# ai4ce/V2X-Sim

Measured on AMD Instinct MI355X. Metric: BEV frames/sec, V2VNet 5-agent detection (256x256 BEV), higher is better.
Workload: dtype bf16

## Files before the change

### v2x-sim_amd/csrc/conv_halo.hip

```cpp
#include "common.h"
#include <cstdlib>

static __device__ __attribute__((aligned(64))) unsigned int g_zero_page_h[16];

typedef const __attribute__((address_space(1))) void *gptr_t;
typedef __attribute__((address_space(3))) void *lptr_t;

__device__ __forceinline__ void glds16h(const void *g, char *lds_wave_base) {
    __builtin_amdgcn_global_load_lds((gptr_t)g, (lptr_t)lds_wave_base, 16, 0, 0);
}

struct HaloArgs {
    const uint16_t *in0;
    const uint16_t *in1;
    const uint32_t *bits;
    int zbits;
    int N, H, W;
    const uint16_t *w;
    const float *scale, *shift;
    int relu;
    void *out;
    int out_cstride, out_coff;
    const uint16_t *w2;
    const float *scale2, *shift2;
// ... 300 lines not shown
            auto hidden = [&](const f32x4_t &lo, const f32x4_t &hi, const float4 &s0, const float4 &t0, const float4 &s1, const float4 &t1) {
                uint4 p;
                p.x = pack_bf16x2(lo[0] * s0.x + t0.x, lo[1] * s0.y + t0.y);
                p.y = pack_bf16x2(lo[2] * s0.z + t0.z, lo[3] * s0.w + t0.w);
                p.z = pack_bf16x2(hi[0] * s1.x + t1.x, hi[1] * s1.y + t1.y);
                p.w = pack_bf16x2(hi[2] * s1.z + t1.z, hi[3] * s1.w + t1.w);
                p.x = v2x_relu_bf16x2_floor(p.x, relu_floor);
                p.y = v2x_relu_bf16x2_floor(p.y, relu_floor);
                p.z = v2x_relu_bf16x2_floor(p.z, relu_floor);
                p.w = v2x_relu_bf16x2_floor(p.w, relu_floor);
                return __builtin_bit_cast(bf16x8_t, p);
            };
            const float4 det_sc0 = *reinterpret_cast<const float4 *>(a.scale + 8 * fq), det_sf0 = *reinterpret_cast<const float4 *>(a.shift + 8 * fq);
            const float4 det_sc1 = *reinterpret_cast<const float4 *>(a.scale + 8 * fq + 4), det_sf1 = *reinterpret_cast<const float4 *>(a.shift + 8 * fq + 4);
            const float4 det_s2 = *reinterpret_cast<const float4 *>(a.scale2 + fq * 4), det_t2 = *reinterpret_cast<const float4 *>(a.shift2 + fq * 4);
            float4 cl[4];
            unsigned long long any_f[4];
#pragma unroll
            for (int f = 0; f < 4; ++f) {
                const bf16x8_t hb0 = hidden(acc[0][f], acc[1][f], det_sc0, det_sf0, det_sc1, det_sf1);
                const f32x4_t d = __builtin_amdgcn_mfma_f32_16x16x32_bf16(wdet[0], hb0, (f32x4_t){0.f, 0.f, 0.f, 0.f}, 0, 0, 0);
                cl[f] = make_float4(d[0] * det_s2.x + det_t2.x, d[1] * det_s2.y + det_t2.y, d[2] * det_s2.z + det_t2.z, d[3] * det_s2.w + det_t2.w);
                const bool maybe = fq < 3 && ((cl[f].y - cl[f].x >= a.det_margin) || (cl[f].w - cl[f].z >= a.det_margin));
                any_f[f] = __builtin_amdgcn_ballot_w64(maybe);
            }
            if ((any_f[0] | any_f[1] | any_f[2] | any_f[3]) != 0) {
                const float4 sc2 = *reinterpret_cast<const float4 *>(a.scale + 32 + 8 * fq), sf2 = *reinterpret_cast<const float4 *>(a.shift + 32 + 8 * fq);
                const float4 sc3 = *reinterpret_cast<const float4 *>(a.scale + 36 + 8 * fq), sf3 = *reinterpret_cast<const float4 *>(a.shift + 36 + 8 * fq);
                float4 s2v[3], t2v[3];
#pragma unroll
                for (int t = 0; t < 3; ++t) {
                    s2v[t] = *reinterpret_cast<const float4 *>(a.scale2 + (t + 1) * 16 + fq * 4);
                    t2v[t] = *reinterpret_cast<const float4 *>(a.shift2 + (t + 1) * 16 + fq * 4);
                }
#pragma unroll
                for (int f = 0; f < 4; ++f) {
                    const float4 c = cl[f];
                    if (any_f[f] == 0) continue;
                    const int r = f >> 1, ch = f & 1;
                    f32x4_t g2 = (f32x4_t){0.f, 0.f, 0.f, 0.f}, g3 = g2;
#pragma unroll
                    for (int kx = 0; kx < 3; ++kx)
#pragma unroll
                        for (int ky = 0; ky < 3; ++ky) {
                            const int kslot = (ky * 3 + kx) * SPP1 + fq;
                            const int pr = 2 * wave + r + ky, pc = ch * 16 + fj + kx;
                            const bf16x8_t Bf = *reinterpret_cast<const bf16x8_t *>(pb + NS0 * 16 + ((pr * PW + pc) * SPP1 + swz<SPP1>(fq, pc)) * 16);
                            const bf16x8_t A2 = *reinterpret_cast<const bf16x8_t *>(s_w + (kslot * COUT + 32 + fj) * 16);
                            const bf16x8_t A3 = *reinterpret_cast<const bf16x8_t *>(s_w + (kslot * COUT + 48 + fj) * 16);
                            g2 = __builtin_amdgcn_mfma_f32_16x16x32_bf16(A2, Bf, g2, 0, 0, 0);
                            g3 = __builtin_amdgcn_mfma_f32_16x16x32_bf16(A3, Bf, g3, 0, 0, 0);
                        }
                    const bf16x8_t hb1 = hidden(g2, g3, sc2, sf2, sc3, sf3);
                    float4 cd[3];
#pragma unroll
                    for (int t = 0; t < 3; ++t) {
                        const f32x4_t e = __builtin_amdgcn_mfma_f32_16x16x32_bf16(wdet[t + 1], hb1, (f32x4_t){0.f, 0.f, 0.f, 0.f}, 0, 0, 0);
                        cd[t] = make_float4(e[0] * s2v[t].x + t2v[t].x, e[1] * s2v[t].y + t2v[t].y, e[2] * s2v[t].z + t2v[t].z, e[3] * s2v[t].w + t2v[t].w);
                    }
                    if (fq < 3) {
                        const int y = ty * TH + 2 * wave + r, x = tx * TW + ch * 16 + fj;
                        const float c0[2] = {c.x, c.z}, c1[2] = {c.y, c.w};
                        const float code[2][6] = {{cd[0].x, cd[0].y, cd[0].z, cd[0].w, cd[1].x, cd[1].y},
                                                  {cd[1].z, cd[1].w, cd[2].x, cd[2].y, cd[2].z, cd[2].w}};
#pragma unroll
                        for (int u = 0; u < 2; ++u) {
                            const float mx = fmaxf(c0[u], c1[u]);
                            const float e0 = expf(c0[u] - mx), e1 = expf(c1[u] - mx);
                            const float fg = e1 / (e0 + e1);
                            if (fg >= a.det_thr) {
                                const int pos = atomicAdd(&a.det_counts[n], 1);
                                if (pos < a.det_cap) {
                                    const unsigned m = (unsigned)((y * a.W + x) * 6 + 2 * fq + u);
                                    reinterpret_cast<unsigned long long *>(a.out)[(size_t)n * a.det_cap + pos] =
                                        ((unsigned long long)(~__float_as_uint(fg)) << 32) | (m << 12) | (unsigned)pos;
                                    float *co = reinterpret_cast<float *>(a.out2) + ((size_t)n * a.det_cap + pos) * 6;
                                    *reinterpret_cast<float2 *>(co) = make_float2(code[u][0], code[u][1]);
                                    *reinterpret_cast<float2 *>(co + 2) = make_float2(code[u][2], code[u][3]);
                                    *reinterpret_cast<float2 *>(co + 4) = make_float2(code[u][4], code[u][5]);
                                }
                            }
                        }
                    }
                }
            }
        } else if constexpr (COUT2 == 0) {
            if (a.x4) {
#pragma unroll
                for (int i = 0; i < TCO; i += 2) {
                    float4 sc[2], sf[2];
#pragma unroll
                    for (int h = 0; h < 2; ++h) {
                        sc[h] = *reinterpret_cast<const float4 *>(s_ss + (i + h) * 16 + fq * 4);
                        sf[h] = *reinterpret_cast<const float4 *>(s_ss + COUT + (i + h) * 16 + fq * 4);
                    }
#pragma unroll
                    for (int f = 0; f < 4; ++f) {
                        const int y = ty * TH + 2 * wave + (f >> 1), x = tx * TW + (f & 1) * 16 + fj;
                        uint32_t ox[2], oy[2];
#pragma unroll
                        for (int h = 0; h < 2; ++h) {
                            ox[h] = v2x_relu_bf16x2_floor(pack_bf16x2(acc[i + h][f][0] * sc[h].x + sf[h].x, acc[i + h][f][1] * sc[h].y + sf[h].y), relu_floor);
                            oy[h] = v2x_relu_bf16x2_floor(pack_bf16x2(acc[i + h][f][2] * sc[h].z + sf[h].z, acc[i + h][f][3] * sc[h].w + sf[h].w), relu_floor);
                        }
                        v2x_store_pair_x4(reinterpret_cast<uint16_t *>(a.out) + ((size_t)(n * a.H + y) * a.W + x) * a.out_cstride + a.out_coff + i * 16 + fq * 4, fq,
                                          ox[0], oy[0], ox[1], oy[1]);
                    }
                }
            } else
#pragma unroll
            for (int i = 0; i < TCO; ++i) {
                const int co = i * 16 + fq * 4;
                const float4 sc = *reinterpret_cast<const float4 *>(s_ss + co);
                const float4 sf = *reinterpret_cast<const float4 *>(s_ss + COUT + co);
#pragma unroll
                for (int f = 0; f < 4; ++f) {
                    const int y = ty * TH + 2 * wave + (f >> 1), x = tx * TW + (f & 1) * 16 + fj;
                    float v0 = acc[i][f][0] * sc.x + sf.x, v1 = acc[i][f][1] * sc.y + sf.y;
                    float v2 = acc[i][f][2] * sc.z + sf.z, v3 = acc[i][f][3] * sc.w + sf.w;
                    uint2 o;
                    o.x = pack_bf16x2(v0, v1);
                    o.y = pack_bf16x2(v2, v3);
                    o.x = v2x_relu_bf16x2_floor(o.x, relu_floor);
                    o.y = v2x_relu_bf16x2_floor(o.y, relu_floor);
                    uint16_t *dst = reinterpret_cast<uint16_t *>(a.out) +
                                    ((size_t)(n * a.H + y) * a.W + x) * a.out_cstride + a.out_coff + co;
                    *reinterpret_cast<uint2 *>(dst) = o;
                }
            }
        } else {
            float4 sc[TCO], sf[TCO];
#pragma unroll
            for (int i = 0; i < TCO; ++i) {
                const int kappa = 32 * (i >> 1) + 8 * fq + 4 * (i & 1);
                sc[i] = *reinterpret_cast<const float4 *>(a.scale + kappa);
                sf[i] = *reinterpret_cast<const float4 *>(a.shift + kappa);
            }
            float4 s2v[TCO2 > 0 ? TCO2 : 1], t2v[TCO2 > 0 ? TCO2 : 1];
#pragma unroll
            for (int i2 = 0; i2 < TCO2; ++i2) {
                s2v[i2] = *reinterpret_cast<const float4 *>(a.scale2 + i2 * 16 + fq * 4);
                t2v[i2] = *reinterpret_cast<const float4 *>(a.shift2 + i2 * 16 + fq * 4);
            }
#pragma unroll
            for (int f = 0; f < 4; ++f) {
                bf16x8_t hb[COUT / 32];
#pragma unroll
                for (int s = 0; s < COUT / 32; ++s) {
                    float h[8];
#pragma unroll
                    for (int half = 0; half < 2; ++half) {
                        const int i = 2 * s + half;
                        h[half * 4 + 0] = acc[i][f][0] * sc[i].x + sf[i].x;
                        h[half * 4 + 1] = acc[i][f][1] * sc[i].y + sf[i].y;
                        h[half * 4 + 2] = acc[i][f][2] * sc[i].z + sf[i].z;
                        h[half * 4 + 3] = acc[i][f][3] * sc[i].w + sf[i].w;
                    }
                    uint4 p;
                    p.x = pack_bf16x2(h[0], h[1]);
                    p.y = pack_bf16x2(h[2], h[3]);
                    p.z = pack_bf16x2(h[4], h[5]);
                    p.w = pack_bf16x2(h[6], h[7]);
                    p.x = v2x_relu_bf16x2_floor(p.x, relu_floor);
                    p.y = v2x_relu_bf16x2_floor(p.y, relu_floor);
                    p.z = v2x_relu_bf16x2_floor(p.z, relu_floor);
                    p.w = v2x_relu_bf16x2_floor(p.w, relu_floor);
                    hb[s] = __builtin_bit_cast(bf16x8_t, p);
                }
                const int y = ty * TH + 2 * wave + (f >> 1), x = tx * TW + (f & 1) * 16 + fj;
                const size_t pix = (size_t)(n * a.H + y) * a.W + x;
#pragma unroll
                for (int i2 = 0; i2 < TCO2; ++i2) {
                    f32x4_t d = (f32x4_t){0.f, 0.f, 0.f, 0.f};
#pragma unroll
                    for (int s = 0; s < COUT / 32; ++s)
                        d = __builtin_amdgcn_mfma_f32_16x16x32_bf16(w2f[i2][s], hb[s], d, 0, 0, 0);
                    const int co = i2 * 16 + fq * 4;
                    if (co >= a.cout2_real) continue;
                    const float4 s2 = s2v[i2], t2 = t2v[i2];
                    float v0 = d[0] * s2.x + t2.x, v1 = d[1] * s2.y + t2.y, v2 = d[2] * s2.z + t2.z, v3 = d[3] * s2.w + t2.w;
                    if (a.relu2) {
                        v0 = fmaxf(v0, 0.f);
                        v1 = fmaxf(v1, 0.f);
                        v2 = fmaxf(v2, 0.f);
                        v3 = fmaxf(v3, 0.f);
                    }
                    if constexpr (EPI2 == 2) {
                        const bool second = a.split > 0 && co >= a.split;
                        float *dst = second ? reinterpret_cast<float *>(a.out2) + pix * a.out2_cstride + (co - a.split)
                                            : reinterpret_cast<float *>(a.out) + pix * a.out_cstride + a.out_coff + co;
                        *reinterpret_cast<float4 *>(dst) = make_float4(v0, v1, v2, v3);
                    } else {
                        uint2 o;
                        o.x = pack_bf16x2(v0, v1);
                        o.y = pack_bf16x2(v2, v3);
                        uint16_t *dst = reinterpret_cast<uint16_t *>(a.out) + pix * a.out_cstride + a.out_coff + co;
                        *reinterpret_cast<uint2 *>(dst) = o;
                    }
                }
            }
        }
        if constexpr (DB) {
            cur ^= 1;
        } else {
            __builtin_amdgcn_s_barrier();
        }
    }
}

template <int C0, int C1, int COUT, int COUT2, int EPI2>
__global__ __launch_bounds__(256) __attribute__((amdgpu_waves_per_eu((C0 == 0 && C1 == 64 && COUT2 == 64) ? 1 : 2, 2))) void conv3x3_halo_kernel(const HaloArgs a) {
    conv3x3_halo_body<C0, C1, COUT, COUT2, EPI2, true>(a);
}

template <int C0, int C1, int COUT, int COUT2, int EPI2, bool BITS>
__global__ __launch_bounds__(256) __attribute__((amdgpu_waves_per_eu(4, 4))) void conv3x3_halo_sb_kernel(const HaloArgs a) {
    conv3x3_halo_body<C0, C1, COUT, COUT2, EPI2, false, BITS>(a);
}

template <int C0, int C1, int COUT, int COUT2 = 0>
__global__ __launch_bounds__(512) __attribute__((amdgpu_waves_per_eu(2, 2))) void conv3x3_halo_pp_kernel(const HaloArgs a) {
    constexpr int SPP0 = C0 / 8, SPP1 = C1 / 8;
    constexpr int NS1 = round64(PH * PW * SPP1);
    constexpr int NS0 = C0 ? round64(PH0 * PW0 * SPP0) : 0;
    constexpr int PATCH_BYTES = (NS0 + NS1) * 16;
    constexpr int KSLOTS = 9 * (SPP0 + SPP1);
    constexpr int W_BYTES = KSLOTS * COUT * 16;
    constexpr int TCO = COUT / 16;
    static_assert(C0 % 32 == 0 && C1 % 32 == 0 && (TCO == 2 || TCO == 4), "ping-pong form: 32 or 64 output channels");
    static_assert(W_BYTES % 1024 == 0, "weights are moved 1 KiB per wave instruction");
    constexpr int TCO2 = COUT2 / 16;
    static_assert(COUT2 == 0 || (COUT2 == 64 && COUT == 64), "chained 1x1: 64 -> 64 (conv1_2 -> conv3d_1)");
    constexpr int N_STORES = (COUT2 ? TCO2 : TCO) * 4;

    extern __shared__ __attribute__((aligned(16))) char smem[];
    const uint32_t relu_floor = a.relu ? 0u : 0x80008000u;
    char *s_w = smem;
    char *s_patch = smem + W_BYTES;
    float *s_ss = reinterpret_cast<float *>(smem + W_BYTES + 2 * PATCH_BYTES);
    for (int i = threadIdx.x; i < COUT; i += 512) {
        s_ss[i] = a.scale[i];
        s_ss[COUT + i] = a.shift[i];
    }
    if constexpr (COUT2 > 0) {
        for (int i = threadIdx.x; i < COUT2; i += 512) {
            s_ss[2 * COUT + i] = a.scale2[i];
            s_ss[2 * COUT + COUT2 + i] = a.shift2[i];
        }
    }

    const int tid = threadIdx.x;
    const int lane = tid & 63;
    const int wave = __builtin_amdgcn_readfirstlane(tid >> 6);
    const int grp = wave >> 2, wv = wave & 3;
    const int fj = lane & 15, fq = lane >> 4;
    char *pb = s_patch + grp * PATCH_BYTES;

    for (int off = wave * 1024; off < W_BYTES; off += 8192)
        glds16h(reinterpret_cast<const char *>(a.w) + off + lane * 16, s_w + off);

    constexpr bool TABLES = (COUT2 == 0);
    constexpr int NP1 = (NS1 + 255) / 256, NP0 = (NS0 + 255) / 256;
    int tb1[TABLES ? NP1 : 1], tb0[NP0 ? NP0 : 1];
#pragma unroll
    for (int t = 0; t < (TABLES ? NP1 : 0); ++t) {
        const int L = wv * 64 + t * 256 + lane;
        const int pix = L / SPP1, phys = L - pix * SPP1;
        const int pr = pix / PW, pc = pix - pr * PW;
        tb1[t] = pix < PH * PW ? (((pr * a.W + pc) * C1 + swz<SPP1>(phys, pc) * 8) | (pr << 20) | (pc << 24)) : -1;
    }
    if constexpr (C0 > 0) {
        constexpr int S0 = SPP0 ? SPP0 : 1;
#pragma unroll
        for (int t = 0; t < NP0; ++t) {
            const int L = wv * 64 + t * 256 + lane;
            const int pix = L / S0, phys = L - pix * S0;
            const int pr = pix / PW0, pc = pix - pr * PW0;
            tb0[t] = pix < PH0 * PW0 ? (((pr * (a.W >> 1) + pc) * C0 + swz<(SPP0 ? SPP0 : 4)>(phys, pc) * 8) | (pr << 20) | (pc << 24)) : -1;
        }
    }

    const int txy = a.tiles_x * a.tiles_y;
    auto coords = [&](int tile, int &n, int &y0, int &x0) {
        n = tile / txy;
        const int r = tile - n * txy;
        const int ty = r / a.tiles_x;
        y0 = ty * TH;
        x0 = (r - ty * a.tiles_x) * TW;
    };
    auto load_patch = [&](int tile) {
        int n, y0, x0;
        coords(tile, n, y0, x0);
        if constexpr (TABLES) {
            const unsigned base = ((unsigned)(n * a.H + y0 - 1) * (unsigned)a.W + (unsigned)(x0 - 1)) * (unsigned)C1;
#pragma unroll
            for (int t = 0; t < NP1; ++t) {
                if (wv * 64 + t * 256 >= NS1) break;
                const int y = y0 - 1 + ((tb1[t] >> 20) & 15), x = x0 - 1 + ((tb1[t] >> 24) & 63);
                const bool ok = tb1[t] >= 0 && (unsigned)y < (unsigned)a.H && (unsigned)x < (unsigned)a.W;
                glds16h(ok ? (const void *)(a.in1 + (base + (unsigned)(tb1[t] & 0xfffff))) : (const void *)g_zero_page_h,
                        pb + NS0 * 16 + (wv * 64 + t * 256) * 16);
            }
        } else {
            for (int base = wv * 64; base < NS1; base += 256) {
                const int L = base + lane;
                const int pix = L / SPP1, phys = L - pix * SPP1;
                const int pr = pix / PW, pc = pix - pr * PW;
                const int y = y0 - 1 + pr, x = x0 - 1 + pc;
                const bool ok = pix < PH * PW && (unsigned)y < (unsigned)a.H && (unsigned)x < (unsigned)a.W;
                const unsigned off = ((unsigned)(n * a.H + y) * (unsigned)a.W + (unsigned)x) * (unsigned)C1 + swz<SPP1>(phys, pc) * 8;
                glds16h(ok ? (const void *)(a.in1 + off) : (const void *)g_zero_page_h, pb + NS0 * 16 + base * 16);
            }
        }
        if constexpr (C0 > 0) {
            const int Hs = a.H >> 1, Ws = a.W >> 1;
            const unsigned base = ((unsigned)(n * Hs + (y0 >> 1) - 1) * (unsigned)Ws + (unsigned)((x0 >> 1) - 1)) * (unsigned)C0;
#pragma unroll
            for (int t = 0; t < NP0; ++t) {
                if (wv * 64 + t * 256 >= NS0) break;
                const int y = (y0 >> 1) - 1 + ((tb0[t] >> 20) & 15), x = (x0 >> 1) - 1 + ((tb0[t] >> 24) & 63);
                const bool ok = tb0[t] >= 0 && (unsigned)y < (unsigned)Hs && (unsigned)x < (unsigned)Ws;
                glds16h(ok ? (const void *)(a.in0 + (base + (unsigned)(tb0[t] & 0xfffff))) : (const void *)g_zero_page_h,
                        pb + (wv * 64 + t * 256) * 16);
            }
        }
    };

    f32x4_t acc[TCO][4];
    constexpr int KC0 = C0 / 32, KC1 = C1 / 32, KC = KC0 + KC1, NG = 3 * KC;
    struct Frags {
        bf16x8_t A[3][TCO];
        bf16x8_t B[8];
    };
    auto load_group = [&](int g, Frags &F) {
        const int kx = g / KC, kk = g - kx * KC;
        if (kk < KC0) {
#pragma unroll
            for (int ky = 0; ky < 3; ++ky) {
                const int kslot = (ky * 3 + kx) * (SPP0 + SPP1) + kk * 4 + fq;
#pragma unroll
                for (int i = 0; i < TCO; ++i)
                    F.A[ky][i] = *reinterpret_cast<const bf16x8_t *>(s_w + (kslot * COUT + i * 16 + fj) * 16);
            }
#pragma unroll
            for (int hr = 0; hr < 3; ++hr)
#pragma unroll
                for (int ch = 0; ch < 2; ++ch) {
                    const int pr = wv + hr;
                    const int pc = ((ch * 16 + fj + kx - 1) >> 1) + 1;
                    F.B[hr * 2 + ch] = *reinterpret_cast<const bf16x8_t *>(pb + ((pr * PW0 + pc) * (SPP0 ? SPP0 : 1) + swz<(SPP0 ? SPP0 : 4)>(kk * 4 + fq, pc)) * 16);
                }
        } else {
            const int kc = kk - KC0;
#pragma unroll
            for (int ky = 0; ky < 3; ++ky) {
                const int kslot = (ky * 3 + kx) * (SPP0 + SPP1) + SPP0 + kc * 4 + fq;
#pragma unroll
                for (int i = 0; i < TCO; ++i)
                    F.A[ky][i] = *reinterpret_cast<const bf16x8_t *>(s_w + (kslot * COUT + i * 16 + fj) * 16);
            }
#pragma unroll
            for (int rr = 0; rr < 4; ++rr)
#pragma unroll
                for (int ch = 0; ch < 2; ++ch) {
                    const int pr = 2 * wv + rr;
                    const int pc = ch * 16 + fj + kx;
                    F.B[rr * 2 + ch] = *reinterpret_cast<const bf16x8_t *>(pb + NS0 * 16 + ((pr * PW + pc) * SPP1 + swz<SPP1>(kc * 4 + fq, pc)) * 16);
                }
        }
    };
    auto mma_group = [&](int g, const Frags &F) {
        const bool half = (g % KC) < KC0;
#pragma unroll
        for (int ky = 0; ky < 3; ++ky)
#pragma unroll
            for (int i = 0; i < TCO; ++i)
#pragma unroll
                for (int f = 0; f < 4; ++f) {
                    const int r = f >> 1, ch = f & 1;
                    const int row = half ? (((r + ky - 1) >> 1) + 1) : (r + ky);
                    acc[i][f] = __builtin_amdgcn_mfma_f32_16x16x32_bf16(F.A[ky][i], F.B[row * 2 + ch], acc[i][f], 0, 0, 0);
                }
    };
    auto compute = [&]() {
#pragma unroll
        for (int i = 0; i < TCO; ++i)
#pragma unroll
            for (int f = 0; f < 4; ++f) acc[i][f] = (f32x4_t){0.f, 0.f, 0.f, 0.f};
        if constexpr (TCO == 2) {
            Frags fr[2];
            load_group(0, fr[0]);
#pragma unroll
            for (int g = 0; g < NG; ++g) {
                if (g + 1 < NG) load_group(g + 1, fr[(g + 1) & 1]);
                __builtin_amdgcn_sched_barrier(0);
                mma_group(g, fr[g & 1]);
                __builtin_amdgcn_sched_barrier(0);
            }
        } else {
            static_assert(C0 == 0 || TCO == 2, "the 64-channel form has one full-resolution source");
            bf16x8_t B[8], A[2][TCO];
            auto load_A = [&](int g, int ky, bf16x8_t (&Ak)[TCO]) {
                const int kx = g / KC, kc = g - kx * KC;
                const int kslot = (ky * 3 + kx) * (SPP0 + SPP1) + SPP0 + kc * 4 + fq;
#pragma unroll
                for (int i = 0; i < TCO; ++i) Ak[i] = *reinterpret_cast<const bf16x8_t *>(s_w + (kslot * COUT + i * 16 + fj) * 16);
            };
#pragma unroll
            for (int g = 0; g < NG; ++g) {
                const int kx = g / KC, kc = g - kx * KC;
#pragma unroll
                for (int rr = 0; rr < 4; ++rr)
#pragma unroll
                    for (int ch = 0; ch < 2; ++ch) {
                        const int pr = 2 * wv + rr, pc = ch * 16 + fj + kx;
                        B[rr * 2 + ch] = *reinterpret_cast<const bf16x8_t *>(pb + NS0 * 16 + ((pr * PW + pc) * SPP1 + swz<SPP1>(kc * 4 + fq, pc)) * 16);
                    }
                load_A(g, 0, A[0]);
#pragma unroll
                for (int ky = 0; ky < 3; ++ky) {
                    if (ky < 2) load_A(g, ky + 1, A[(ky + 1) & 1]);
                    __builtin_amdgcn_sched_barrier(0);
#pragma unroll
                    for (int i = 0; i < TCO; ++i)
#pragma unroll
                        for (int f = 0; f < 4; ++f)
                            acc[i][f] = __builtin_amdgcn_mfma_f32_16x16x32_bf16(A[ky & 1][i], B[((f >> 1) + ky) * 2 + (f & 1)], acc[i][f], 0, 0, 0);
                    __builtin_amdgcn_sched_barrier(0);
                }
            }
        }
    };
    auto epilogue = [&](int tile) {
        int n, y0, x0;
        coords(tile, n, y0, x0);
        int zo = 0;
        asm volatile("" : "+v"(zo));
        const float *ss = s_ss + zo;
        if constexpr (COUT2 > 0) {
            bf16x8_t w2f[TCO2][COUT / 32];
            int w2off = fj * COUT + fq * 8;
            asm volatile("" : "+v"(w2off));
#pragma unroll
            for (int i2 = 0; i2 < TCO2; ++i2)
#pragma unroll
                for (int ks = 0; ks < COUT / 32; ++ks)
                    w2f[i2][ks] = *reinterpret_cast<const bf16x8_t *>(a.w2 + w2off + i2 * 16 * COUT + ks * 32);
            asm volatile("s_waitcnt vmcnt(0)" ::: "memory");
#pragma unroll
            for (int f = 0; f < 4; ++f) {
                bf16x8_t hb[COUT / 32];
#pragma unroll
                for (int ks = 0; ks < COUT / 32; ++ks) {
                    float h[8];
#pragma unroll
                    for (int hf = 0; hf < 2; ++hf) {
                        const int i = 2 * ks + hf;
                        const int kappa = 32 * (i >> 1) + 8 * fq + 4 * (i & 1);
                        const float4 sc = *reinterpret_cast<const float4 *>(ss + kappa);
                        const float4 sf = *reinterpret_cast<const float4 *>(ss + COUT + kappa);
                        h[hf * 4 + 0] = acc[i][f][0] * sc.x + sf.x;
                        h[hf * 4 + 1] = acc[i][f][1] * sc.y + sf.y;
                        h[hf * 4 + 2] = acc[i][f][2] * sc.z + sf.z;
                        h[hf * 4 + 3] = acc[i][f][3] * sc.w + sf.w;
                    }
                    uint4 p;
                    p.x = pack_bf16x2(h[0], h[1]);
                    p.y = pack_bf16x2(h[2], h[3]);
                    p.z = pack_bf16x2(h[4], h[5]);
                    p.w = pack_bf16x2(h[6], h[7]);
                    p.x = v2x_relu_bf16x2_floor(p.x, relu_floor);
                    p.y = v2x_relu_bf16x2_floor(p.y, relu_floor);
                    p.z = v2x_relu_bf16x2_floor(p.z, relu_floor);
                    p.w = v2x_relu_bf16x2_floor(p.w, relu_floor);
                    hb[ks] = __builtin_bit_cast(bf16x8_t, p);
                }
                const int y = y0 + 2 * wv + (f >> 1), x = x0 + (f & 1) * 16 + fj;
                uint16_t *prow = reinterpret_cast<uint16_t *>(a.out) + ((size_t)(n * a.H + y) * a.W + x) * a.out_cstride + a.out_coff;
                if (a.x4) {
                    const uint32_t floor2 = a.relu2 ? 0u : 0x80008000u;
#pragma unroll
                    for (int i2 = 0; i2 + 1 < TCO2; i2 += 2) {
                        uint32_t ox[2], oy[2];
#pragma unroll
                        for (int h = 0; h < 2; ++h) {
                            const int co = (i2 + h) * 16 + fq * 4;
                            const float4 s2 = *reinterpret_cast<const float4 *>(ss + 2 * COUT + co);
                            const float4 t2 = *reinterpret_cast<const float4 *>(ss + 2 * COUT + COUT2 + co);
                            f32x4_t d = (f32x4_t){0.f, 0.f, 0.f, 0.f};
#pragma unroll
                            for (int ks = 0; ks < COUT / 32; ++ks) d = __builtin_amdgcn_mfma_f32_16x16x32_bf16(w2f[i2 + h][ks], hb[ks], d, 0, 0, 0);
                            ox[h] = v2x_relu_bf16x2_floor(pack_bf16x2(d[0] * s2.x + t2.x, d[1] * s2.y + t2.y), floor2);
                            oy[h] = v2x_relu_bf16x2_floor(pack_bf16x2(d[2] * s2.z + t2.z, d[3] * s2.w + t2.w), floor2);
                        }
                        v2x_store_pair_x4(prow + i2 * 16 + fq * 4, fq, ox[0], oy[0], ox[1], oy[1]);
                    }
                    continue;
                }
#pragma unroll
                for (int i2 = 0; i2 < TCO2; ++i2) {
                    const int co = i2 * 16 + fq * 4;
                    const float4 s2 = *reinterpret_cast<const float4 *>(ss + 2 * COUT + co);
                    const float4 t2 = *reinterpret_cast<const float4 *>(ss + 2 * COUT + COUT2 + co);
                    f32x4_t d = (f32x4_t){0.f, 0.f, 0.f, 0.f};
#pragma unroll
                    for (int ks = 0; ks < COUT / 32; ++ks) d = __builtin_amdgcn_mfma_f32_16x16x32_bf16(w2f[i2][ks], hb[ks], d, 0, 0, 0);
                    float v0 = d[0] * s2.x + t2.x, v1 = d[1] * s2.y + t2.y, v2 = d[2] * s2.z + t2.z, v3 = d[3] * s2.w + t2.w;
                    if (a.relu2) {
                        v0 = fmaxf(v0, 0.f);
                        v1 = fmaxf(v1, 0.f);
                        v2 = fmaxf(v2, 0.f);
                        v3 = fmaxf(v3, 0.f);
                    }
                    uint2 o;
                    o.x = pack_bf16x2(v0, v1);
                    o.y = pack_bf16x2(v2, v3);
                    *reinterpret_cast<uint2 *>(prow + co) = o;
                }
            }
            return;
        }
        if (a.x4) {
#pragma unroll
            for (int i = 0; i < TCO; i += 2) {
                float4 sc[2], sf[2];
#pragma unroll
                for (int h = 0; h < 2; ++h) {
                    sc[h] = *reinterpret_cast<const float4 *>(ss + (i + h) * 16 + fq * 4);
                    sf[h] = *reinterpret_cast<const float4 *>(ss + COUT + (i + h) * 16 + fq * 4);
                }
#pragma unroll
                for (int f = 0; f < 4; ++f) {
                    const int y = y0 + 2 * wv + (f >> 1), x = x0 + (f & 1) * 16 + fj;
                    uint32_t ox[2], oy[2];
#pragma unroll
                    for (int h = 0; h < 2; ++h) {
                        ox[h] = v2x_relu_bf16x2_floor(pack_bf16x2(acc[i + h][f][0] * sc[h].x + sf[h].x, acc[i + h][f][1] * sc[h].y + sf[h].y), relu_floor);
                        oy[h] = v2x_relu_bf16x2_floor(pack_bf16x2(acc[i + h][f][2] * sc[h].z + sf[h].z, acc[i + h][f][3] * sc[h].w + sf[h].w), relu_floor);
                    }
                    v2x_store_pair_x4(reinterpret_cast<uint16_t *>(a.out) + ((size_t)(n * a.H + y) * a.W + x) * a.out_cstride + a.out_coff + i * 16 + fq * 4, fq,
                                      ox[0], oy[0], ox[1], oy[1]);
                }
            }
            return;
        }
#pragma unroll
        for (int i = 0; i < TCO; ++i) {
            const int co = i * 16 + fq * 4;
            const float4 sc = *reinterpret_cast<const float4 *>(ss + co);
            const float4 sf = *reinterpret_cast<const float4 *>(ss + COUT + co);
#pragma unroll
            for (int f = 0; f < 4; ++f) {
                const int y = y0 + 2 * wv + (f >> 1), x = x0 + (f & 1) * 16 + fj;
                float v0 = acc[i][f][0] * sc.x + sf.x, v1 = acc[i][f][1] * sc.y + sf.y;
                float v2 = acc[i][f][2] * sc.z + sf.z, v3 = acc[i][f][3] * sc.w + sf.w;
                uint2 o;
                o.x = pack_bf16x2(v0, v1);
                o.y = pack_bf16x2(v2, v3);
                o.x = v2x_relu_bf16x2_floor(o.x, relu_floor);
                o.y = v2x_relu_bf16x2_floor(o.y, relu_floor);
                uint16_t *dst = reinterpret_cast<uint16_t *>(a.out) + ((size_t)(n * a.H + y) * a.W + x) * a.out_cstride + a.out_coff + co;
                *reinterpret_cast<uint2 *>(dst) = o;
            }
        }
    };

    const int n_pairs = a.n_tiles >> 1;
    const v2x_tile_walk walk = v2x_xcd_tile_walk(n_pairs, a.xcd_walk);
    const int K = walk.first < walk.end ? (walk.end - walk.first + walk.step - 1) / walk.step : 0;
    auto tile_of = [&](int k) { return 2 * (walk.first + k * walk.step) + grp; };

    if (grp == 0) load_patch(tile_of(0));
    __syncthreads();

    for (int i = 0; i <= 2 * K; ++i) {
        if ((i & 1) == grp) {
            if ((i >> 1) < K) compute();
        } else {
            const int m = (i - grp - 1) / 2;
            if (m + 1 < K) load_patch(tile_of(m + 1));
            if (m >= 0) {
                epilogue(tile_of(m));
                if constexpr (N_STORES == 8) {
                    if (a.x4) asm volatile("s_waitcnt vmcnt(4)" ::: "memory");
                    else asm volatile("s_waitcnt vmcnt(8)" ::: "memory");
                } else {
                    if (a.x4) asm volatile("s_waitcnt vmcnt(8)" ::: "memory");
                    else asm volatile("s_waitcnt vmcnt(16)" ::: "memory");
                }
            } else {
                asm volatile("s_waitcnt vmcnt(0)" ::: "memory");
            }
        }
        __builtin_amdgcn_sched_barrier(0);
        __builtin_amdgcn_s_barrier();
        __builtin_amdgcn_sched_barrier(0);
    }
    static_assert(N_STORES == 8 || N_STORES == 16, "the counted waits above know 8 or 16 stores per tile and wave");
}

template <int C0, int C1, int COUT, int COUT2 = 0>
static int launch_halo_pp(const HaloArgs &a, hipStream_t s) {
    constexpr int NS1 = round64(PH * PW * (C1 / 8));
    constexpr int NS0 = C0 ? round64(PH0 * PW0 * (C0 / 8)) : 0;
    constexpr int smem = 9 * (C0 + C1) / 8 * COUT * 16 + 2 * (NS0 + NS1) * 16 + 2 * COUT * 4 + 2 * COUT2 * 4;
    static_assert(smem <= 160 * 1024, "LDS budget");
    int grid = 256;
    if (grid > a.n_tiles / 2) grid = a.n_tiles / 2;
    return v2x_launch<conv3x3_halo_pp_kernel<C0, C1, COUT, COUT2>>("conv3x3_halo_pp_kernel", dim3(grid), dim3(512), smem, s, a);
}

constexpr int PWH = PW / 2;

template <int C0, int C1, int COUT>
__global__ __launch_bounds__(512) __attribute__((amdgpu_waves_per_eu(2, 2))) void conv3x3_halo_ppc_kernel(const HaloArgs a) {
    constexpr int SPP0 = C0 / 8, SPP1 = C1 / 8;
    constexpr int NS1 = round64(2 * PH * PWH * SPP1);
    constexpr int NS0 = round64(PH0 * PW0 * SPP0);
    constexpr int PATCH_BYTES = (NS0 + NS1) * 16;
    constexpr int W_UP_BYTES = 16 * SPP0 * COUT * 16;
    constexpr int W_BYTES = W_UP_BYTES + 9 * SPP1 * COUT * 16;
    constexpr int TCO = COUT / 16;
    constexpr int KC0 = C0 / 32, KC1 = C1 / 32;
    static_assert(C0 % 32 == 0 && C1 % 32 == 0 && C0 > 0 && C1 > 0 && TCO == 2, "parity-class form: two sources, 32 output channels");
    static_assert(W_BYTES % 1024 == 0, "weights are moved 1 KiB per wave instruction");
    constexpr int N_STORES = TCO * 4;

    extern __shared__ __attribute__((aligned(16))) char smem[];
    const uint32_t relu_floor = a.relu ? 0u : 0x80008000u;
    char *s_w = smem;
    char *s_patch = smem + W_BYTES;
    float *s_ss = reinterpret_cast<float *>(smem + W_BYTES + 2 * PATCH_BYTES);
    for (int i = threadIdx.x; i < COUT; i += 512) {
        s_ss[i] = a.scale[i];
        s_ss[COUT + i] = a.shift[i];
    }

    const int tid = threadIdx.x;
    const int lane = tid & 63;
    const int wave = __builtin_amdgcn_readfirstlane(tid >> 6);
    const int grp = wave >> 2, wv = wave & 3;
    const int py = wv >> 1, px = wv & 1;
    const int fj = lane & 15, fq = lane >> 4;
    char *pb = s_patch + grp * PATCH_BYTES;

    for (int off = wave * 1024; off < W_BYTES; off += 8192)
        glds16h(reinterpret_cast<const char *>(a.w) + off + lane * 16, s_w + off);

    constexpr int NP1 = (NS1 + 255) / 256, NP0 = (NS0 + 255) / 256;
    int tb1[NP1], tb0[NP0];
#pragma unroll
    for (int t = 0; t < NP1; ++t) {
        const int L = wv * 64 + t * 256 + lane;
        const int pix = L / SPP1, phys = L - pix * SPP1;
        const int q = pix / (PH * PWH), rem = pix - q * (PH * PWH);
        const int pr = rem / PWH, cc = rem - pr * PWH;
        const int pc = 2 * cc + q;
        tb1[t] = pix < 2 * PH * PWH ? (((pr * a.W + pc) * C1 + swz<SPP1>(phys, cc) * 8) | (pr << 20) | (pc << 24)) : -1;
    }
#pragma unroll
    for (int t = 0; t < NP0; ++t) {
        const int L = wv * 64 + t * 256 + lane;
        const int pix = L / SPP0, phys = L - pix * SPP0;
        const int pr = pix / PW0, pc = pix - pr * PW0;
        tb0[t] = pix < PH0 * PW0 ? (((pr * (a.W >> 1) + pc) * C0 + swz<SPP0>(phys, pc) * 8) | (pr << 20) | (pc << 24)) : -1;
    }

    const int txy = a.tiles_x * a.tiles_y;
    auto coords = [&](int tile, int &n, int &y0, int &x0) {
        n = tile / txy;
        const int r = tile - n * txy;
        const int ty = r / a.tiles_x;
        y0 = ty * TH;
        x0 = (r - ty * a.tiles_x) * TW;
    };
    auto load_patch = [&](int tile) {
        int n, y0, x0;
        coords(tile, n, y0, x0);
        {
            const unsigned base = ((unsigned)(n * a.H + y0 - 1) * (unsigned)a.W + (unsigned)(x0 - 1)) * (unsigned)C1;
#pragma unroll
            for (int t = 0; t < NP1; ++t) {
                if (wv * 64 + t * 256 >= NS1) break;
                const int y = y0 - 1 + ((tb1[t] >> 20) & 15), x = x0 - 1 + ((tb1[t] >> 24) & 63);
                const bool ok = tb1[t] >= 0 && (unsigned)y < (unsigned)a.H && (unsigned)x < (unsigned)a.W;
                glds16h(ok ? (const void *)(a.in1 + (base + (unsigned)(tb1[t] & 0xfffff))) : (const void *)g_zero_page_h,
                        pb + NS0 * 16 + (wv * 64 + t * 256) * 16);
            }
        }
        {
            const int Hs = a.H >> 1, Ws = a.W >> 1;
            const unsigned base = ((unsigned)(n * Hs + (y0 >> 1) - 1) * (unsigned)Ws + (unsigned)((x0 >> 1) - 1)) * (unsigned)C0;
#pragma unroll
            for (int t = 0; t < NP0; ++t) {
                if (wv * 64 + t * 256 >= NS0) break;
                const int y = (y0 >> 1) - 1 + ((tb0[t] >> 20) & 15), x = (x0 >> 1) - 1 + ((tb0[t] >> 24) & 63);
                const bool ok = tb0[t] >= 0 && (unsigned)y < (unsigned)Hs && (unsigned)x < (unsigned)Ws;
                glds16h(ok ? (const void *)(a.in0 + (base + (unsigned)(tb0[t] & 0xfffff))) : (const void *)g_zero_page_h,
                        pb + (wv * 64 + t * 256) * 16);
            }
        }
    };

    f32x4_t acc[TCO][4];
    constexpr int NG = 2 * KC0 + 3 * KC1;
    struct Frags {
        bf16x8_t A[3 * TCO];
        bf16x8_t B[9];
    };
    auto load_group = [&](int g, Frags &F) {
        if (g < 2 * KC0) {
            const int kc = g >> 1, b = g & 1;
#pragma unroll
            for (int t = 0; t < 2; ++t)
#pragma unroll
                for (int i = 0; i < TCO; ++i)
                    F.A[t * TCO + i] = *reinterpret_cast<const bf16x8_t *>(s_w + ((((wv * 4 + t * 2 + b) * SPP0 + kc * 4 + fq) * COUT) + i * 16 + fj) * 16);
            const int pc = fj + b + px;
#pragma unroll
            for (int r = 0; r < 5; ++r)
                F.B[r] = *reinterpret_cast<const bf16x8_t *>(pb + (((py + r) * PW0 + pc) * SPP0 + swz<SPP0>(kc * 4 + fq, pc)) * 16);
        } else {
            const int h = g - 2 * KC0, kx = h / KC1, kc = h - kx * KC1;
#pragma unroll
            for (int ky = 0; ky < 3; ++ky)
#pragma unroll
                for (int i = 0; i < TCO; ++i)
                    F.A[ky * TCO + i] = *reinterpret_cast<const bf16x8_t *>(s_w + W_UP_BYTES + ((((ky * 3 + kx) * SPP1 + kc * 4 + fq) * COUT) + i * 16 + fj) * 16);
            const int q = (px + kx) & 1, cc = fj + ((px + kx) >> 1);
#pragma unroll
            for (int r = 0; r < 9; ++r)
                F.B[r] = *reinterpret_cast<const bf16x8_t *>(pb + NS0 * 16 + ((((q * PH) + py + r) * PWH + cc) * SPP1 + swz<SPP1>(kc * 4 + fq, cc)) * 16);
        }
    };
    auto mma_group = [&](int g, const Frags &F) {
        if (g < 2 * KC0) {
#pragma unroll
            for (int t = 0; t < 2; ++t)
#pragma unroll
                for (int i = 0; i < TCO; ++i)
#pragma unroll
                    for (int f = 0; f < 4; ++f) acc[i][f] = __builtin_amdgcn_mfma_f32_16x16x32_bf16(F.A[t * TCO + i], F.B[f + t], acc[i][f], 0, 0, 0);
        } else {
#pragma unroll
            for (int ky = 0; ky < 3; ++ky)
#pragma unroll
                for (int i = 0; i < TCO; ++i)
#pragma unroll
                    for (int f = 0; f < 4; ++f) acc[i][f] = __builtin_amdgcn_mfma_f32_16x16x32_bf16(F.A[ky * TCO + i], F.B[2 * f + ky], acc[i][f], 0, 0, 0);
        }
    };
    auto compute = [&]() {
#pragma unroll
        for (int i = 0; i < TCO; ++i)
#pragma unroll
            for (int f = 0; f < 4; ++f) acc[i][f] = (f32x4_t){0.f, 0.f, 0.f, 0.f};
        Frags fr[2];
        load_group(0, fr[0]);
#pragma unroll
        for (int g = 0; g < NG; ++g) {
            if (g + 1 < NG) load_group(g + 1, fr[(g + 1) & 1]);
            __builtin_amdgcn_sched_barrier(0);
            mma_group(g, fr[g & 1]);
            __builtin_amdgcn_sched_barrier(0);
        }
    };
    auto epilogue = [&](int tile) {
        int n, y0, x0;
        coords(tile, n, y0, x0);
        int zo = 0;
        asm volatile("" : "+v"(zo));
        const float *ss = s_ss + zo;
        float4 sc[2], sf[2];
#pragma unroll
        for (int h = 0; h < 2; ++h) {
            sc[h] = *reinterpret_cast<const float4 *>(ss + h * 16 + fq * 4);
            sf[h] = *reinterpret_cast<const float4 *>(ss + COUT + h * 16 + fq * 4);
        }
#pragma unroll
        for (int f = 0; f < 4; ++f) {
            const int y = y0 + 2 * f + py, x = x0 + 2 * fj + px;
            uint32_t ox[2], oy[2];
#pragma unroll
            for (int h = 0; h < 2; ++h) {
                ox[h] = v2x_relu_bf16x2_floor(pack_bf16x2(acc[h][f][0] * sc[h].x + sf[h].x, acc[h][f][1] * sc[h].y + sf[h].y), relu_floor);
                oy[h] = v2x_relu_bf16x2_floor(pack_bf16x2(acc[h][f][2] * sc[h].z + sf[h].z, acc[h][f][3] * sc[h].w + sf[h].w), relu_floor);
            }
            uint16_t *prow = reinterpret_cast<uint16_t *>(a.out) + ((size_t)(n * a.H + y) * a.W + x) * a.out_cstride + a.out_coff + fq * 4;
            if (a.x4) {
                v2x_store_pair_x4(prow, fq, ox[0], oy[0], ox[1], oy[1]);
            } else {
                *reinterpret_cast<uint2 *>(prow) = make_uint2(ox[0], oy[0]);
                *reinterpret_cast<uint2 *>(prow + 16) = make_uint2(ox[1], oy[1]);
            }
        }
    };

    const int n_pairs = (a.n_tiles + 1) >> 1;
    const v2x_tile_walk walk = v2x_xcd_tile_walk(n_pairs, a.xcd_walk);
    const int K = walk.first < walk.end ? (walk.end - walk.first + walk.step - 1) / walk.step : 0;
    auto tile_of = [&](int k) { return 2 * (walk.first + k * walk.step) + grp; };
    auto has = [&](int k) { return k < K && tile_of(k) < a.n_tiles; };

    if (grp == 0 && has(0)) load_patch(tile_of(0));
    __syncthreads();

    for (int i = 0; i <= 2 * K; ++i) {
        if ((i & 1) == grp) {
            if (has(i >> 1)) compute();
        } else {
            const int m = (i - grp - 1) / 2;
            if (has(m + 1)) load_patch(tile_of(m + 1));
            if (m >= 0 && has(m)) {
                epilogue(tile_of(m));
                if (a.x4) asm volatile("s_waitcnt vmcnt(4)" ::: "memory");
                else asm volatile("s_waitcnt vmcnt(8)" ::: "memory");
            } else {
                asm volatile("s_waitcnt vmcnt(0)" ::: "memory");
            }
        }
        __builtin_amdgcn_sched_barrier(0);
        __builtin_amdgcn_s_barrier();
        __builtin_amdgcn_sched_barrier(0);
    }
    static_assert(N_STORES == 8, "the counted waits above know 8 (4 in the 16-byte form) stores per tile and wave");
}

template <int C0, int C1, int COUT>
static int launch_halo_ppc(const HaloArgs &a, hipStream_t s) {
    constexpr int NS1 = round64(2 * PH * PWH * (C1 / 8));
    constexpr int NS0 = round64(PH0 * PW0 * (C0 / 8));
    constexpr int smem = (16 * C0 + 9 * C1) / 8 * COUT * 16 + 2 * (NS0 + NS1) * 16 + 2 * COUT * 4;
    static_assert(smem <= 160 * 1024, "LDS budget");
    int grid = 256;
    if (grid > (a.n_tiles + 1) / 2) grid = (a.n_tiles + 1) / 2;
    return v2x_launch<conv3x3_halo_ppc_kernel<C0, C1, COUT>>("conv3x3_halo_ppc_kernel", dim3(grid), dim3(512), smem, s, a);
}

template <int C0, int C1, int COUT, int COUT2, int EPI2, bool BITS>
static int launch_halo_sb(const HaloArgs &a, hipStream_t s) {
    static_assert(C0 == 0, "single-buffer form: one source");
    constexpr int smem = 9 * C1 / 8 * COUT * 16 + (BITS ? PH * PW * (C1 / 8) : round64(PH * PW * (C1 / 8))) * 16 +
                         (COUT2 == 0 ? 2 * COUT * 4 : 0);
    int per_cu = (160 * 1024 - 2048) / smem;
    if (per_cu > 4) per_cu = 4;
    if (per_cu < 1) per_cu = 1;
    int grid = 256 * per_cu;
    if (grid > a.n_tiles) grid = a.n_tiles;
    return v2x_launch<conv3x3_halo_sb_kernel<C0, C1, COUT, COUT2, EPI2, BITS>>("conv3x3_halo_sb_kernel", dim3(grid), dim3(256), smem, s, a);
}

template <int C0, int C1, int COUT, int COUT2, int EPI2>
static int launch_halo(const HaloArgs &a, hipStream_t s) {
    constexpr int NS1 = round64(PH * PW * (C1 / 8));
    constexpr int NS0 = C0 ? round64(PH0 * PW0 * (C0 / 8)) : 0;
    constexpr int smem = 9 * (C0 + C1) / 8 * COUT * 16 + 2 * (NS0 + NS1) * 16 + (COUT2 == 0 ? 2 * COUT * 4 : 0);
    static_assert(smem <= 160 * 1024, "LDS budget");
    const int per_cu = (160 * 1024) / smem >= 2 ? 2 : 1;
    int grid = 256 * per_cu;
    if (grid > a.n_tiles) grid = a.n_tiles;
    return v2x_launch<conv3x3_halo_kernel<C0, C1, COUT, COUT2, EPI2>>("conv3x3_halo_kernel", dim3(grid), dim3(256), smem, s, a);
}

int v2x_conv_halo_dispatch(const v2x_conv_desc *d, hipStream_t s) {
    HaloArgs a;
    a.xcd_walk = v2x_tune(V2X_TUNE_HALO_XCD);
    a.x4 = (d->epilogue == V2X_EPI_BF16) ? v2x_x4_ok(d->out, d->out_cstride, d->out_coff, d->Cout2 > 0 ? d->Cout2 : d->Cout) : 0;
    a.in0 = d->C1 ? d->in0 : nullptr;
    a.in1 = d->C1 ? d->in1 : d->in0;
    a.bits = d->in_format == 1 ? reinterpret_cast<const uint32_t *>(d->in0) : nullptr;
    a.zbits = d->in_zbits;
    const int C0 = d->C1 ? d->C0 : 0, C1 = d->C1 ? d->C1 : d->C0;
    a.N = d->N;
    a.H = d->H;
    a.W = d->W;
    a.w = d->weight;
    a.scale = d->scale;
    a.shift = d->shift;
    a.relu = d->relu;
    a.out = d->out;
    a.out_cstride = d->out_cstride;
    a.out_coff = d->out_coff;
    a.w2 = d->weight2;
    a.scale2 = d->scale2;
    a.shift2 = d->shift2;
    a.relu2 = d->relu2;
    a.cout2_real = d->Cout2;
    a.split = d->split;
    a.out2 = d->out2;
    a.out2_cstride = d->out2_cstride;
    a.det_counts = d->det_counts;
    a.det_thr = d->det_thr;
    {
        const double t = d->det_thr;
        if (t <= 0.0) a.det_margin = -3.0e38f;
        else if (t >= 1.0) a.det_margin = 16.0f;
        else {
            const double slack = fmax(1e-3, 4e-7 / (t * (1.0 - t)));
            a.det_margin = (float)fmin(log(t / (1.0 - t)) - slack, 16.0);
        }
    }
    a.det_cap = d->det_cap;
    {
        const int cmax = d->C1 ? (d->C0 > d->C1 ? d->C0 : d->C1) : d->C0;
        if ((long long)(PH * d->W + PW) * cmax >= (1 << 20)) return 1;
    }
    a.tiles_x = d->W / TW;
    a.tiles_y = d->H / TH;
    a.n_tiles = d->N * a.tiles_x * a.tiles_y;
    const int co2 = d->Cout2 > 0 ? (d->Cout2 + 15) / 16 * 16 : 0;
    const int e2 = d->Cout2 > 0 ? (d->epilogue == V2X_EPI_DET ? 3 : (d->epilogue == V2X_EPI_F32 ? 2 : 1)) : 0;
#define HALO_CASE(c0, c1, co, c2, ep) \
    if (C0 == c0 && C1 == c1 && d->Cout == co && co2 == c2 && e2 == ep) return launch_halo<c0, c1, co, c2, ep>(a, s);
    if (C0 == 0 && C1 == 32 && d->Cout == 32 && co2 == 0 && e2 == 0)
        return d->in_format == 1 ? launch_halo_sb<0, 32, 32, 0, 0, true>(a, s) : launch_halo_sb<0, 32, 32, 0, 0, false>(a, s);
    if (d->in_format == 1) return 1;
    if (d->w_layout == 3) {
        if (C0 == 64 && C1 == 32 && d->Cout == 32 && co2 == 0 && e2 == 0) return launch_halo_ppc<64, 32, 32>(a, s);
        return 1;
    }
    if (C0 == 64 && C1 == 32 && d->Cout == 32 && co2 == 0 && e2 == 0 && a.n_tiles >= 2 && a.n_tiles % 2 == 0) {
        if (v2x_tune(V2X_TUNE_HALO_PP) != 0) return launch_halo_pp<64, 32, 32>(a, s);
    }
    HALO_CASE(64, 32, 32, 0, 0)
    if (C0 == 0 && C1 == 64 && d->Cout == 64 && co2 == 0 && e2 == 0 && a.n_tiles >= 2 && a.n_tiles % 2 == 0) {
        if (v2x_tune(V2X_TUNE_HALO_PP) != 0) return launch_halo_pp<0, 64, 64>(a, s);
    }
    HALO_CASE(0, 64, 64, 0, 0)
    if (C0 == 0 && C1 == 64 && d->Cout == 64 && co2 == 64 && e2 == 1 && d->Cout2 == 64 && a.n_tiles >= 2 && a.n_tiles % 2 == 0 &&
        d->split == 0)
        return launch_halo_pp<0, 64, 64, 64>(a, s);
    HALO_CASE(0, 64, 64, 64, 1)
    HALO_CASE(0, 64, 32, 0, 0)
    HALO_CASE(0, 32, 64, 0, 0)
    HALO_CASE(0, 32, 64, 48, 2)
    HALO_CASE(0, 32, 32, 16, 2)
    if (e2 == 3) {
        if (!(C0 == 0 && C1 == 32 && d->Cout == 64 && d->Cout2 == 64 && d->det_counts && d->out && d->out2 && d->det_cap > 0 &&
              d->det_cap <= 4096 && (long long)d->H * d->W * 6 < (1 << 20)))
            return 1;
        return launch_halo<0, 32, 64, 64, 3>(a, s);
    }
#undef HALO_CASE
    return 1;
}
```

Baseline: 6588.

## Prefetch chained-conv weights and scales before patch DMA in ping-pong halo kernel

```diff
diff --git a/v2x-sim_amd/csrc/conv_halo.hip b/v2x-sim_amd/csrc/conv_halo.hip
--- a/v2x-sim_amd/csrc/conv_halo.hip
+++ b/v2x-sim_amd/csrc/conv_halo.hip
@@ -626,14 +626,30 @@
                         pb + NS0 * 16 + (wv * 64 + t * 256) * 16);
             }
         } else {
-            for (int base = wv * 64; base < NS1; base += 256) {
-                const int L = base + lane;
-                const int pix = L / SPP1, phys = L - pix * SPP1;
-                const int pr = pix / PW, pc = pix - pr * PW;
+            constexpr int STEP = 256 / SPP1;
+            static_assert(256 % SPP1 == 0 && STEP <= PW, "the incremental (pr, pc) walk below");
+            const int L0 = wv * 64 + lane;
+            int pix = L0 / SPP1;
+            const int phys = L0 - pix * SPP1;
+            int pr = pix / PW, pc = pix - pr * PW;
+            unsigned row = (unsigned)(n * a.H + y0 - 1 + pr) * (unsigned)a.W + (unsigned)(x0 - 1);
+            const void *zero_page = g_zero_page_h;
+            asm volatile("" : "+s"(zero_page));
+#pragma unroll 1
+            for (int t = 0; t < NP1; ++t) {
+                const int base = wv * 64 + t * 256;
+                if (base >= NS1) break;
                 const int y = y0 - 1 + pr, x = x0 - 1 + pc;
                 const bool ok = pix < PH * PW && (unsigned)y < (unsigned)a.H && (unsigned)x < (unsigned)a.W;
-                const unsigned off = ((unsigned)(n * a.H + y) * (unsigned)a.W + (unsigned)x) * (unsigned)C1 + swz<SPP1>(phys, pc) * 8;
-                glds16h(ok ? (const void *)(a.in1 + off) : (const void *)g_zero_page_h, pb + NS0 * 16 + base * 16);
+                const unsigned off = (row + (unsigned)pc) * (unsigned)C1 + swz<SPP1>(phys, pc) * 8;
+                glds16h(ok ? (const void *)(a.in1 + off) : zero_page, pb + NS0 * 16 + base * 16);
+                pix += STEP;
+                pc += STEP;
+                if (pc >= PW) {
+                    pc -= PW;
+                    ++pr;
+                    row += (unsigned)a.W;
+                }
             }
         }
         if constexpr (C0 > 0) {
@@ -755,22 +771,63 @@
             }
         }
     };
-    auto epilogue = [&](int tile) {
+    struct ChainOps {
+        bf16x8_t f[TCO2 ? TCO2 : 1][COUT / 32];
+        f32x4_t sc1[4], sf1[4];
+        f32x4_t sc2[4], sf2[4];
+    };
+    auto load_chain_ops = [&](ChainOps &c) {
+        int w2off = fj * COUT + fq * 8, zo = 0;
+        asm volatile("" : "+v"(w2off), "+v"(zo));
+        const uint16_t *p = a.w2 + w2off;
+#pragma unroll
+        for (int i2 = 0; i2 < TCO2; ++i2)
+#pragma unroll
+            for (int ks = 0; ks < COUT / 32; ++ks)
+                asm volatile("global_load_dwordx4 %0, %1, off offset:%2"
+                             : "=v"(c.f[i2][ks])
+                             : "v"(p + (i2 >> 1) * 32 * COUT), "n"(((i2 & 1) * 16 * COUT + ks * 32) * 2)
+                             : "memory");
+        static_assert(COUT2 == 0 || (COUT == 64 && COUT2 == 64), "the LDS offsets below are those of [scale | shift | scale2 | shift2], 64 floats each");
+        const uint32_t ss_lds = (uint32_t)(uintptr_t)(__attribute__((address_space(3))) const float *)(s_ss + zo);
+        const uint32_t a1 = ss_lds + fq * 32, a2 = ss_lds + fq * 16;
+        asm volatile("ds_read_b128 %0, %16\n\t"
+                     "ds_read_b128 %1, %16 offset:16\n\t"
+                     "ds_read_b128 %2, %16 offset:128\n\t"
+                     "ds_read_b128 %3, %16 offset:144\n\t"
+                     "ds_read_b128 %4, %16 offset:256\n\t"
+                     "ds_read_b128 %5, %16 offset:272\n\t"
+                     "ds_read_b128 %6, %16 offset:384\n\t"
+                     "ds_read_b128 %7, %16 offset:400\n\t"
+                     "ds_read_b128 %8, %17 offset:512\n\t"
+                     "ds_read_b128 %9, %17 offset:576\n\t"
+                     "ds_read_b128 %10, %17 offset:640\n\t"
+                     "ds_read_b128 %11, %17 offset:704\n\t"
+                     "ds_read_b128 %12, %17 offset:768\n\t"
+                     "ds_read_b128 %13, %17 offset:832\n\t"
+                     "ds_read_b128 %14, %17 offset:896\n\t"
+                     "ds_read_b128 %15, %17 offset:960"
+                     : "=&v"(c.sc1[0]), "=&v"(c.sc1[1]), "=&v"(c.sc1[2]), "=&v"(c.sc1[3]), "=&v"(c.sf1[0]), "=&v"(c.sf1[1]), "=&v"(c.sf1[2]), "=&v"(c.sf1[3]),
+                       "=&v"(c.sc2[0]), "=&v"(c.sc2[1]), "=&v"(c.sc2[2]), "=&v"(c.sc2[3]), "=&v"(c.sf2[0]), "=&v"(c.sf2[1]), "=&v"(c.sf2[2]), "=&v"(c.sf2[3])
+                     : "v"(a1), "v"(a2)
+                     : "memory");
+    };
+    auto pin_chain_ops = [&](ChainOps &c) {
+#pragma unroll
+        for (int i2 = 0; i2 < TCO2; ++i2)
+#pragma unroll
+            for (int ks = 0; ks < COUT / 32; ++ks) asm volatile("" : "+v"(c.f[i2][ks]));
+#pragma unroll
+        for (int i = 0; i < 4; ++i) asm volatile("" : "+v"(c.sc1[i]), "+v"(c.sf1[i]), "+v"(c.sc2[i]), "+v"(c.sf2[i]));
+    };
+    auto epilogue = [&](int tile, const ChainOps &w2) {
         int n, y0, x0;
         coords(tile, n, y0, x0);
         int zo = 0;
         asm volatile("" : "+v"(zo));
         const float *ss = s_ss + zo;
         if constexpr (COUT2 > 0) {
-            bf16x8_t w2f[TCO2][COUT / 32];
-            int w2off = fj * COUT + fq * 8;
-            asm volatile("" : "+v"(w2off));
-#pragma unroll
-            for (int i2 = 0; i2 < TCO2; ++i2)
-#pragma unroll
-                for (int ks = 0; ks < COUT / 32; ++ks)
-                    w2f[i2][ks] = *reinterpret_cast<const bf16x8_t *>(a.w2 + w2off + i2 * 16 * COUT + ks * 32);
-            asm volatile("s_waitcnt vmcnt(0)" ::: "memory");
+            const f32x4_t(&sc1)[4] = w2.sc1, (&sf1)[4] = w2.sf1, (&sc2)[4] = w2.sc2, (&sf2)[4] = w2.sf2;
 #pragma unroll
             for (int f = 0; f < 4; ++f) {
                 bf16x8_t hb[COUT / 32];
@@ -780,9 +837,7 @@
 #pragma unroll
                     for (int hf = 0; hf < 2; ++hf) {
                         const int i = 2 * ks + hf;
-                        const int kappa = 32 * (i >> 1) + 8 * fq + 4 * (i & 1);
-                        const float4 sc = *reinterpret_cast<const float4 *>(ss + kappa);
-                        const float4 sf = *reinterpret_cast<const float4 *>(ss + COUT + kappa);
+                        const f32x4_t sc = sc1[i], sf = sf1[i];
                         h[hf * 4 + 0] = acc[i][f][0] * sc.x + sf.x;
                         h[hf * 4 + 1] = acc[i][f][1] * sc.y + sf.y;
                         h[hf * 4 + 2] = acc[i][f][2] * sc.z + sf.z;
@@ -799,6 +854,13 @@
                     p.w = v2x_relu_bf16x2_floor(p.w, relu_floor);
                     hb[ks] = __builtin_bit_cast(bf16x8_t, p);
                 }
+                f32x4_t d2[TCO2];
+#pragma unroll
+                for (int i2 = 0; i2 < TCO2; ++i2) d2[i2] = (f32x4_t){0.f, 0.f, 0.f, 0.f};
+#pragma unroll
+                for (int ks = 0; ks < COUT / 32; ++ks)
+#pragma unroll
+                    for (int i2 = 0; i2 < TCO2; ++i2) d2[i2] = __builtin_amdgcn_mfma_f32_16x16x32_bf16(w2.f[i2][ks], hb[ks], d2[i2], 0, 0, 0);
                 const int y = y0 + 2 * wv + (f >> 1), x = x0 + (f & 1) * 16 + fj;
                 uint16_t *prow = reinterpret_cast<uint16_t *>(a.out) + ((size_t)(n * a.H + y) * a.W + x) * a.out_cstride + a.out_coff;
                 if (a.x4) {
@@ -808,12 +870,8 @@
                         uint32_t ox[2], oy[2];
 #pragma unroll
                         for (int h = 0; h < 2; ++h) {
-                            const int co = (i2 + h) * 16 + fq * 4;
-                            const float4 s2 = *reinterpret_cast<const float4 *>(ss + 2 * COUT + co);
-                            const float4 t2 = *reinterpret_cast<const float4 *>(ss + 2 * COUT + COUT2 + co);
-                            f32x4_t d = (f32x4_t){0.f, 0.f, 0.f, 0.f};
-#pragma unroll
-                            for (int ks = 0; ks < COUT / 32; ++ks) d = __builtin_amdgcn_mfma_f32_16x16x32_bf16(w2f[i2 + h][ks], hb[ks], d, 0, 0, 0);
+                            const f32x4_t s2 = sc2[i2 + h], t2 = sf2[i2 + h];
+                            const f32x4_t d = d2[i2 + h];
                             ox[h] = v2x_relu_bf16x2_floor(pack_bf16x2(d[0] * s2.x + t2.x, d[1] * s2.y + t2.y), floor2);
                             oy[h] = v2x_relu_bf16x2_floor(pack_bf16x2(d[2] * s2.z + t2.z, d[3] * s2.w + t2.w), floor2);
                         }
@@ -824,11 +882,8 @@
 #pragma unroll
                 for (int i2 = 0; i2 < TCO2; ++i2) {
                     const int co = i2 * 16 + fq * 4;
-                    const float4 s2 = *reinterpret_cast<const float4 *>(ss + 2 * COUT + co);
-                    const float4 t2 = *reinterpret_cast<const float4 *>(ss + 2 * COUT + COUT2 + co);
-                    f32x4_t d = (f32x4_t){0.f, 0.f, 0.f, 0.f};
-#pragma unroll
-                    for (int ks = 0; ks < COUT / 32; ++ks) d = __builtin_amdgcn_mfma_f32_16x16x32_bf16(w2f[i2][ks], hb[ks], d, 0, 0, 0);
+                    const f32x4_t s2 = sc2[i2], t2 = sf2[i2];
+                    const f32x4_t d = d2[i2];
                     float v0 = d[0] * s2.x + t2.x, v1 = d[1] * s2.y + t2.y, v2 = d[2] * s2.z + t2.z, v3 = d[3] * s2.w + t2.w;
                     if (a.relu2) {
                         v0 = fmaxf(v0, 0.f);
@@ -902,9 +957,19 @@
             if ((i >> 1) < K) compute();
         } else {
             const int m = (i - grp - 1) / 2;
-            if (m + 1 < K) load_patch(tile_of(m + 1));
+            const bool more = m + 1 < K;
+            ChainOps w2;
+            if constexpr (COUT2 > 0) load_chain_ops(w2);
+            if (more) load_patch(tile_of(m + 1));
             if (m >= 0) {
-                epilogue(tile_of(m));
+                if constexpr (COUT2 > 0) {
+                    static_assert(TABLES || (3 * 64 + (NP1 - 2) * 256 < NS1 && C0 == 0), "every wave issues NP1 or NP1 - 1 patch DMAs");
+                    if (!more) asm volatile("s_waitcnt vmcnt(0) lgkmcnt(0)" ::: "memory");
+                    else if (wv * 64 + (NP1 - 1) * 256 < NS1) asm volatile("s_waitcnt vmcnt(%0) lgkmcnt(0)" ::"n"(NP1) : "memory");
+                    else asm volatile("s_waitcnt vmcnt(%0) lgkmcnt(0)" ::"n"(NP1 - 1) : "memory");
+                    pin_chain_ops(w2);
+                }
+                epilogue(tile_of(m), w2);
                 if constexpr (N_STORES == 8) {
                     if (a.x4) asm volatile("s_waitcnt vmcnt(4)" ::: "memory");
                     else asm volatile("s_waitcnt vmcnt(8)" ::: "memory");
@@ -1252,8 +1317,9 @@
     }
     HALO_CASE(0, 64, 64, 0, 0)
     if (C0 == 0 && C1 == 64 && d->Cout == 64 && co2 == 64 && e2 == 1 && d->Cout2 == 64 && a.n_tiles >= 2 && a.n_tiles % 2 == 0 &&
-        d->split == 0)
-        return launch_halo_pp<0, 64, 64, 64>(a, s);
+        d->split == 0) {
+        if (v2x_tune(V2X_TUNE_HALO_PP) != 0) return launch_halo_pp<0, 64, 64, 64>(a, s);
+    }
     HALO_CASE(0, 64, 64, 64, 1)
     HALO_CASE(0, 64, 32, 0, 0)
     HALO_CASE(0, 32, 64, 0, 0)
```

After: 6564. About the same (-0.4%).
